# KimmiShi/TorchDistPackage

Measured on AMD Instinct MI355X. Metric: tokens_per_second, higher is better.
Workload: dtype bf16; 1 GPU; model=gpt2_1.3b, global_batch=16, seq_len=1024, parallelism=dp1_pp1_tp1

## Files before the change

torchdistpackage_amd/ops/__init__.py:

```python

from __future__ import annotations

import contextlib
import math
import os
from typing import Optional

import torch

_EXT = None
_EXT_ERR: Optional[str] = None


def _load_extension():
    global _EXT, _EXT_ERR
    if _EXT is not None or _EXT_ERR is not None:
        return _EXT
    import glob
    import importlib.util
    here = os.path.dirname(os.path.abspath(__file__))
    cands = glob.glob(os.path.join(here, "_tdpa_hip*.so"))
    if not cands:
        _EXT_ERR = (f"in-tree HIP extension not found under {here}; "
                    "run `python -m torchdistpackage_amd.ops.build` "
# ... 344 lines not shown
            lse = torch.logsumexp(s, dim=-1)
            p = torch.softmax(s, dim=-1)
            o = torch.matmul(p, vf).to(q.dtype)
        ctx.save_for_backward(q, k, v, o, lse)
        ctx.causal = causal
        ctx.scale = scale
        return o

    @staticmethod
    def backward(ctx, do):
        q, k, v, o, lse = ctx.saved_tensors
        H, Hkv = q.shape[1], k.shape[1]
        rep = H // Hkv
        if q.is_cuda:
            dq = torch.empty(q.shape, dtype=q.dtype, device=q.device)
            dk = torch.empty(q.shape, dtype=k.dtype, device=k.device)
            dv = torch.empty(q.shape, dtype=v.dtype, device=v.device)
            dq, dk, dv = ext("flash_attention").attn_bwd(
                do.contiguous(), q, k, v, o, lse, dq, dk, dv,
                ctx.causal, ctx.scale)
            if rep > 1:
                B, _, S, D = q.shape
                dk = dk.view(B, Hkv, rep, S, D).sum(2).to(k.dtype)
                dv = dv.view(B, Hkv, rep, S, D).sum(2).to(v.dtype)
        else:
            qf = q.float()
            kf = k.float() if rep == 1 else \
                k.float().repeat_interleave(rep, 1)
            vf = v.float() if rep == 1 else \
                v.float().repeat_interleave(rep, 1)
            dof = do.float()
            s = torch.matmul(qf, kf.transpose(-1, -2)) * ctx.scale
            if ctx.causal:
                S = q.shape[-2]
                mask = torch.ones(S, k.shape[-2], dtype=torch.bool,
                                  device=q.device).tril_()
                s = s.masked_fill(~mask, float("-inf"))
            p = torch.softmax(s, dim=-1)
            dv = torch.matmul(p.transpose(-1, -2), dof)
            dp = torch.matmul(dof, vf.transpose(-1, -2))
            d = (dp * p).sum(-1, keepdim=True)
            ds = p * (dp - d) * ctx.scale
            dq = torch.matmul(ds, kf)
            dk = torch.matmul(ds.transpose(-1, -2), qf)
            if rep > 1:
                B, _, S, D = q.shape
                dk = dk.view(B, Hkv, rep, S, D).sum(2)
                dv = dv.view(B, Hkv, rep, S, D).sum(2)
            dq, dk, dv = dq.to(q.dtype), dk.to(k.dtype), dv.to(v.dtype)
        return dq, dk, dv, None, None


_ATTN_KNOBS = ("dq_recompute", "no_tr16", "pstore", "force_v1",
               "max_ds_bytes")


def attention_knobs() -> dict:
    return dict(zip(_ATTN_KNOBS, ext("attention_knobs").attn_knobs()))


@contextlib.contextmanager
def attention_route(**knobs):
    unknown = set(knobs) - set(_ATTN_KNOBS)
    if unknown:
        raise TypeError(f"unknown attention knob(s) {sorted(unknown)}; "
                        f"known: {_ATTN_KNOBS}")
    e = ext("attention_knobs")
    cur = attention_knobs()
    cur.update(knobs)
    prev = e.attn_set_knobs(*(cur[n] for n in _ATTN_KNOBS))
    try:
        yield
    finally:
        e.attn_set_knobs(*prev)


_warned_hd = set()


def flash_attention(q, k, v, causal: bool = True, scale: float = None):
    D = q.shape[-1]
    if q.is_cuda and D not in (64, 128):
        if D not in _warned_hd:
            _warned_hd.add(D)
            print(f"[tdpa.ops] flash_attention: head_dim {D} has no HIP "
                  f"kernel (64/128 do); using composite SDPA for it")
        rep = q.shape[1] // k.shape[1]
        kk = k if rep == 1 else k.repeat_interleave(rep, 1)
        vv = v if rep == 1 else v.repeat_interleave(rep, 1)
        if scale is None:
            scale = 1.0 / math.sqrt(D)
        return torch.nn.functional.scaled_dot_product_attention(
            q, kk, vv, is_causal=causal, scale=scale)
    return _FlashAttentionFn.apply(q, k, v, causal, scale)



def fused_adamw_(param: torch.Tensor, grad: torch.Tensor,
                 exp_avg: torch.Tensor, exp_avg_sq: torch.Tensor,
                 step: int, lr: float, beta1: float, beta2: float,
                 eps: float, weight_decay: float):
    if param.is_cuda:
        ext("fused_adamw").adamw_step(param, grad, exp_avg, exp_avg_sq,
                                      step, lr, beta1, beta2, eps,
                                      weight_decay)
        return
    bc1 = 1 - beta1 ** step
    bc2 = 1 - beta2 ** step
    param.mul_(1 - lr * weight_decay)
    exp_avg.mul_(beta1).add_(grad, alpha=1 - beta1)
    exp_avg_sq.mul_(beta2).addcmul_(grad, grad, value=1 - beta2)
    denom = (exp_avg_sq / bc2).sqrt_().add_(eps)
    param.addcdiv_(exp_avg, denom, value=-lr / bc1)


def ema_update_(ema: torch.Tensor, param: torch.Tensor, decay: float):
    if ema.is_cuda:
        ext("ema_update").ema_update(ema, param.contiguous(), decay)
        return
    ema.lerp_(param.to(ema.dtype), 1.0 - decay)

# ... 381 lines not shown
```

torchdistpackage_amd/ops/csrc/attention.hip:

```cpp

#include <torch/extension.h>
#include <ATen/hip/HIPContext.h>
#include "common.h"
#include "attn_knobs.h"
#include <cstdlib>
#include <string>
#include <tuple>

namespace {

typedef __attribute__((ext_vector_type(8))) __bf16 bf16x8_v;
typedef __attribute__((ext_vector_type(4))) float f32x4;

constexpr int WQ = 16;
constexpr int KT = 32;
constexpr int NW_FWD = 16;
constexpr int NW_DQ = 8;
constexpr int NW_DKDV = 8;

struct Strides {
  long b, h, s;
};

DEVINL bf16x8_v pack8(const unsigned short* p) {
// ... 576 lines not shown
              " must be on q's device ", q.device(), ", got ", t.device());
  TORCH_CHECK(t.scalar_type() == torch::kBFloat16, fn, ": ", name,
              " must be bf16, got ", t.scalar_type());
  TORCH_CHECK(t.dim() == 4 && t.size(0) == B && t.size(1) == Hh &&
                  t.size(2) == S && t.size(3) == D,
              fn, ": ", name, " must be (", B, ", ", Hh, ", ", S, ", ", D,
              "), got ", t.sizes());
  TORCH_CHECK(t.stride(3) == 1, fn, ": ", name,
              " must have a contiguous last dim, got stride ", t.stride(3));
  for (int d = 0; d < 3; ++d)
    TORCH_CHECK(t.size(d) == 1 || t.stride(d) % 8 == 0, fn, ": ", name,
                " stride ", t.stride(d), " of dim ", d, " is not a multiple "
                "of 8 elements: the kernels use 16-byte vector accesses");
  TORCH_CHECK(reinterpret_cast<uintptr_t>(t.data_ptr()) % 16 == 0, fn, ": ",
              name, " is not 16-byte aligned: the kernels use 16-byte vector "
              "accesses");
}

std::tuple<int64_t, int64_t, int64_t, int64_t, int64_t> check_qkv(
    const char* fn, const torch::Tensor& q, const torch::Tensor& k,
    const torch::Tensor& v) {
  TORCH_CHECK(q.is_cuda() && q.scalar_type() == torch::kBFloat16, fn,
              ": bf16 CUDA tensors required");
  TORCH_CHECK(q.dim() == 4, fn, ": q must be (B, H, S, D), got ", q.sizes());
  const int64_t B = q.size(0), H = q.size(1), S = q.size(2), D = q.size(3);
  TORCH_CHECK(D == 64 || D == 128, fn, ": head_dim must be 64 or 128, got ",
              D);
  TORCH_CHECK(B >= 1 && H >= 1 && S >= 1, fn,
              ": empty problem (S = 0?), q is ", q.sizes());
  TORCH_CHECK(k.dim() == 4 && v.dim() == 4, fn,
              ": k and v must be (B, Hkv, S, D), got ", k.sizes(), " and ",
              v.sizes());
  const int64_t Hkv = k.size(1);
  TORCH_CHECK(Hkv >= 1 && H % Hkv == 0, fn,
              ": n_head must be a multiple of n_kv_head, got ", H, " and ",
              Hkv);
  TORCH_CHECK(k.size(2) == S, fn,
              ": cross-attention S_kv != S_q not supported yet (k has ",
              k.size(2), " keys, q ", S, " rows)");
  check_operand(fn, "q", q, q, B, H, S, D);
  check_operand(fn, "k", k, q, B, Hkv, S, D);
  check_operand(fn, "v", v, q, B, Hkv, S, D);
  return {B, H, Hkv, S, D};
}

}

AttnKnobs& attn_knobs_ref() {
  static AttnKnobs k{
      std::getenv("TDPA_DQ_RECOMPUTE") != nullptr,
      std::getenv("TDPA_NO_TR16") != nullptr,
      std::getenv("TDPA_PSTORE") != nullptr,
      std::getenv("TDPA_ATTN_V1") != nullptr,
      (int64_t)4 << 30};
  return k;
}

using KnobTuple = std::tuple<bool, bool, bool, bool, int64_t>;

KnobTuple attn_knobs() {
  const AttnKnobs& k = attn_knobs_ref();
  return {k.dq_recompute, k.no_tr16, k.pstore, k.force_v1, k.max_ds_bytes};
}

KnobTuple attn_set_knobs(bool dq_recompute, bool no_tr16, bool pstore,
                         bool force_v1, int64_t max_ds_bytes) {
  KnobTuple prev = attn_knobs();
  attn_knobs_ref() =
      AttnKnobs{dq_recompute, no_tr16, pstore, force_v1, max_ds_bytes};
  return prev;
}

std::string attn_bwd_route(int64_t B, int64_t H, int64_t S, int64_t D) {
  const AttnBwdRoute r = attn_bwd_select(attn_knobs_ref(), B, H, S, D);
  if (r.v1) return "v1";
  if (r.recompute) return "v2_recompute";
  std::string name = "v2_workspace";
  if (r.pstore) name += "+pstore";
  if (r.no_tr16) name += "+no_tr16";
  return name;
}

void attn_fwd_v2(torch::Tensor q, torch::Tensor k, torch::Tensor v,
                 torch::Tensor o, torch::Tensor lse, bool causal,
                 double scale);
void attn_bwd_dq_v2(torch::Tensor dout, torch::Tensor q, torch::Tensor k,
                    torch::Tensor v, torch::Tensor lse, torch::Tensor delta,
                    torch::Tensor dq, bool causal, double scale);
void attn_bwd_v2_all(torch::Tensor dout, torch::Tensor q, torch::Tensor k,
                     torch::Tensor v, torch::Tensor lse, torch::Tensor delta,
                     torch::Tensor dq, torch::Tensor dk, torch::Tensor dv,
                     bool causal, double scale, const AttnBwdRoute& route);
void attn_bwd_dkdv_v2(torch::Tensor dout, torch::Tensor q, torch::Tensor k,
                      torch::Tensor v, torch::Tensor lse, torch::Tensor delta,
                      torch::Tensor dk, torch::Tensor dv, bool causal,
                      double scale);

std::vector<torch::Tensor> attn_fwd(torch::Tensor q, torch::Tensor k,
                                    torch::Tensor v, torch::Tensor o,
                                    bool causal, double scale) {
  auto [B_, H_, Hkv_, S_, D_] = check_qkv("attn_fwd", q, k, v);
  check_operand("attn_fwd", "o", o, q, B_, H_, S_, D_);
  const int B = B_, H = H_, S = S_, D = D_, Hkv = Hkv_;
  const int q_per_kv = H / Hkv;
  auto lse = torch::empty({B, H, S}, q.options().dtype(torch::kFloat));
  const bool force_v1 = attn_knobs_ref().force_v1;
  if (D == 128 && !force_v1) {
    attn_fwd_v2(q, k, v, o, lse, causal, scale);
    return {o, lse};
  }
  auto stream = at::cuda::getCurrentHIPStream();
  constexpr int QT = NW_FWD * WQ;
  dim3 grid((S + QT - 1) / QT, B * H), block(NW_FWD * 64);
  Strides qs = get_strides(q), ks = get_strides(k), vs = get_strides(v),
          os = get_strides(o);
  const unsigned short* qp = (const unsigned short*)q.data_ptr();
  const unsigned short* kp = (const unsigned short*)k.data_ptr();
  const unsigned short* vp = (const unsigned short*)v.data_ptr();
  unsigned short* op = (unsigned short*)o.data_ptr();
  float* lp = lse.data_ptr<float>();
#define LAUNCH(DD, CC)                                                        \
  hipLaunchKernelGGL((attn_fwd_kernel<DD, CC, NW_FWD>), grid, block, 0,       \
                     stream, qp, kp, vp, op, lp, qs, ks, vs, os, B, H, S,     \
                     (float)scale, q_per_kv)
  if (D == 128) { if (causal) LAUNCH(128, true); else LAUNCH(128, false); }
  else          { if (causal) LAUNCH(64, true);  else LAUNCH(64, false);  }
#undef LAUNCH
  HIP_CHECK_LAST();
  return {o, lse};
}

std::vector<torch::Tensor> attn_bwd(torch::Tensor dout, torch::Tensor q,
                                    torch::Tensor k, torch::Tensor v,
                                    torch::Tensor o, torch::Tensor lse,
                                    torch::Tensor dq, torch::Tensor dk,
                                    torch::Tensor dv,
                                    bool causal, double scale) {
  auto [B_, H_, Hkv_, S_, D_] = check_qkv("attn_bwd", q, k, v);
  const int B = B_, H = H_, S = S_, D = D_, Hkv = Hkv_;
  const int q_per_kv = H / Hkv;
  check_operand("attn_bwd", "dout", dout, q, B, H, S, D);
  check_operand("attn_bwd", "o", o, q, B, H, S, D);
  check_operand("attn_bwd", "dq", dq, q, B, H, S, D);
  TORCH_CHECK(dk.dim() == 4 && dv.dim() == 4 && dk.size(1) == H &&
                  dv.size(1) == H,
// ... 2 lines not shown
  check_operand("attn_bwd", "dk", dk, q, B, H, S, D);
  check_operand("attn_bwd", "dv", dv, q, B, H, S, D);
  TORCH_CHECK(lse.is_cuda() && lse.device() == q.device() &&
                  lse.scalar_type() == torch::kFloat && lse.dim() == 3 &&
                  lse.size(0) == B && lse.size(1) == H && lse.size(2) == S &&
                  lse.is_contiguous(),
              "attn_bwd: lse must be a contiguous fp32 (", B, ", ", H, ", ",
              S, ") tensor on q's device, got ", lse.scalar_type(), " ",
              lse.sizes(), " strides ", lse.strides(), " on ", lse.device());
  auto delta = torch::empty({B, H, S}, q.options().dtype(torch::kFloat));
  auto stream = at::cuda::getCurrentHIPStream();
  Strides qs = get_strides(q), ks = get_strides(k), vs = get_strides(v),
          os = get_strides(o), dos = get_strides(dout),
          dqs = get_strides(dq), dks = get_strides(dk), dvs = get_strides(dv);

  launch_attn_delta(o, dout, delta, os, dos, B, H, S, D, stream);

  const AttnBwdRoute route = attn_bwd_select(attn_knobs_ref(), B, H, S, D);
  if (!route.v1) {
    attn_bwd_v2_all(dout, q, k, v, lse, delta, dq, dk, dv, causal, scale,
                    route);
    HIP_CHECK_LAST();
    return {dq, dk, dv};
  }
  constexpr int QT_DQ = NW_DQ * WQ;
  constexpr int QT_KV = NW_DKDV * WQ;
  dim3 grid_dq((S + QT_DQ - 1) / QT_DQ, B * H), block_dq(NW_DQ * 64);
  dim3 grid_kv((S + QT_KV - 1) / QT_KV, B * H), block_kv(NW_DKDV * 64);
  const unsigned short* qp = (const unsigned short*)q.data_ptr();
  const unsigned short* kp = (const unsigned short*)k.data_ptr();
  const unsigned short* vp = (const unsigned short*)v.data_ptr();
  const unsigned short* dop = (const unsigned short*)dout.data_ptr();
  const float* lp = lse.data_ptr<float>();
  const float* delp = delta.data_ptr<float>();
#define LAUNCH_BWD(DD, CC)                                                    \
  do {                                                                        \
    hipLaunchKernelGGL((attn_bwd_dq_kernel<DD, CC, NW_DQ>), grid_dq,         \
                       block_dq, 0, stream, qp, kp, vp, dop, lp, delp,        \
                       (unsigned short*)dq.data_ptr(), qs, ks, vs, dos, dqs,  \
                       B, H, S, (float)scale, q_per_kv);                      \
    hipLaunchKernelGGL((attn_bwd_dkdv_kernel<DD, CC, NW_DKDV>), grid_kv,      \
                       block_kv, 0, stream, qp, kp, vp, dop, lp, delp,        \
                       (unsigned short*)dk.data_ptr(),                        \
                       (unsigned short*)dv.data_ptr(), qs, ks, vs, dos,       \
                       dks, dvs, B, H, S, (float)scale, q_per_kv);            \
  } while (0)
  if (D == 128) { if (causal) LAUNCH_BWD(128, true); else LAUNCH_BWD(128, false); }
  else          { if (causal) LAUNCH_BWD(64, true);  else LAUNCH_BWD(64, false);  }
#undef LAUNCH_BWD
  HIP_CHECK_LAST();
  return {dq, dk, dv};
}

torch::Tensor attn_delta(torch::Tensor o, torch::Tensor dout) {
  TORCH_CHECK(o.is_cuda() && o.scalar_type() == torch::kBFloat16 &&
                  o.dim() == 4,
              "attn_delta: o must be a (B, H, S, D) bf16 device tensor");
  const int64_t B = o.size(0), H = o.size(1), S = o.size(2), D = o.size(3);
  TORCH_CHECK(D == 64 || D == 128,
              "attn_delta: head_dim must be 64 or 128, got ", D);
  TORCH_CHECK(B >= 1 && H >= 1 && S >= 1, "attn_delta: empty problem, o is ",
              o.sizes());
  check_operand("attn_delta", "o", o, o, B, H, S, D);
  check_operand("attn_delta", "dout", dout, o, B, H, S, D);
  auto delta = torch::empty({B, H, S}, o.options().dtype(torch::kFloat));
  launch_attn_delta(o, dout, delta, get_strides(o), get_strides(dout), (int)B,
                    (int)H, (int)S, (int)D, at::cuda::getCurrentHIPStream());
  HIP_CHECK_LAST();
  return delta;
}
```

torchdistpackage_amd/ops/csrc/attention_v2.hip:

```cpp

#include <torch/extension.h>
#include <ATen/hip/HIPContext.h>
#include "common.h"
#include "attn_knobs.h"

namespace {

typedef __attribute__((ext_vector_type(8))) __bf16 bf16x8_v;
typedef __attribute__((ext_vector_type(16))) float f32x16;

constexpr int D2 = 128;
constexpr int QW = 32;
constexpr int NW2 = 8;
constexpr int QT2 = NW2 * QW;
constexpr int KV = 64;

struct Strides2 {
  long b, h, s;
};

DEVINL bf16x8_v pack8v(const unsigned short* p) {
  return *(const bf16x8_v*)p;
}

// ... 700 lines not shown
      }
    }
  }
}

}

void attn_bwd_dkdv_v2(torch::Tensor dout, torch::Tensor q, torch::Tensor k,
                      torch::Tensor v, torch::Tensor lse, torch::Tensor delta,
                      torch::Tensor dk, torch::Tensor dv, bool causal,
                      double scale) {
  const int B = q.size(0), H = q.size(1), S = q.size(2), D = q.size(3);
  const int Hkv = k.size(1);
  const int q_per_kv = H / Hkv;
  TORCH_CHECK(D == 128);
  auto get = [](const torch::Tensor& t) {
    return Strides2{t.stride(0), t.stride(1), t.stride(2)};
  };
  auto stream = at::cuda::getCurrentHIPStream();
  dim3 grid((S + QT2 - 1) / QT2, B * H), block(512);
#define L_KV2(CC, WDS, DSP, SPAD, PW, PM1, PM2)                               \
  do {                                                                        \
    hipLaunchKernelGGL((attn_bwd_dkdv_v2_kernel<CC, false, false, PM1>),      \
                       grid, block, 0,                                        \
                       stream, (const unsigned short*)q.data_ptr(),           \
                       (const unsigned short*)k.data_ptr(),                   \
                       (const unsigned short*)v.data_ptr(),                   \
                       (const unsigned short*)dout.data_ptr(),                \
                       lse.data_ptr<float>(), delta.data_ptr<float>(),        \
                       (unsigned short*)dv.data_ptr(), nullptr, 0, PW,        \
                       get(q),                                                \
                       get(k), get(v), get(dout), get(dv), B, H, S,           \
                       (float)scale, q_per_kv);                               \
    hipLaunchKernelGGL((attn_bwd_dkdv_v2_kernel<CC, true, WDS, PM2>),         \
                       grid, block, 0,                                        \
                       stream, (const unsigned short*)q.data_ptr(),           \
                       (const unsigned short*)k.data_ptr(),                   \
                       (const unsigned short*)v.data_ptr(),                   \
                       (const unsigned short*)dout.data_ptr(),                \
                       lse.data_ptr<float>(), delta.data_ptr<float>(),        \
                       (unsigned short*)dk.data_ptr(), DSP, SPAD, PW,         \
                       get(q),                                                \
                       get(k), get(v), get(dout), get(dk), B, H, S,           \
                       (float)scale, q_per_kv);                               \
  } while (0)
  if (causal) L_KV2(true, false, nullptr, 0, nullptr, 0, 0);
  else L_KV2(false, false, nullptr, 0, nullptr, 0, 0);
  HIP_CHECK_LAST();
}


namespace {

template <bool CAUSAL>
__launch_bounds__(512)
__global__ void attn_bwd_dq_lite_kernel(
    const unsigned short* __restrict__ k,
    const unsigned short* __restrict__ dsb,
    unsigned short* __restrict__ dq,
    Strides2 ks, Strides2 dqs,
    int B, int H, int S, long spad, int q_per_kv) {
  __shared__ __attribute__((aligned(16))) unsigned short kt_lds[2][D2 * KV];

  const int bh = blockIdx.y;
  const int bb = bh / H, hh = bh % H;
  const int hkv = hh / q_per_kv;
  const int qtile = CAUSAL ? (gridDim.x - 1 - blockIdx.x) : blockIdx.x;
  const int qbase = qtile * QT2;
  if (qbase >= S) return;
  const int tid = threadIdx.x;
  const int wid = tid / WAVE;
  const int lane = tid % WAVE;
  const int l31 = lane & 31;
  const int hi = lane >> 5;

  const unsigned short* kp = k + bb * ks.b + hkv * ks.h;
  const int qrow = qbase + wid * QW + l31;
  const unsigned short* dsp = dsb +
      ((long)bh * S + (qrow < S ? qrow : S - 1)) * spad;

  f32x16 acc[4];
#pragma unroll
  for (int ds = 0; ds < 4; ++ds) acc[ds] = (f32x16)(0.f);

  const int kv_end = CAUSAL ? min(S, qbase + QT2) : S;

  bf16x8_v k_reg[2];
  auto load_regs = [&](int kt0) {
#pragma unroll
    for (int c = 0; c < 2; ++c) {
      int idx = tid * 8 + c * 4096;
      int gkey = kt0 + idx / D2;
      k_reg[c] = gkey < S ? pack8v(kp + (long)gkey * ks.s + idx % D2)
                          : (bf16x8_v)(__bf16)0.f;
    }
  };
  auto stage_kt = [&](int b) {
#pragma unroll
    for (int c = 0; c < 2; ++c) {
      int idx = tid * 8 + c * 4096;
      int key = idx / D2;
      int col = idx % D2;
      const unsigned short* ksrc = (const unsigned short*)&k_reg[c];
#pragma unroll
      for (int j = 0; j < 8; ++j)
        kt_lds[b][swzV(col + j, key)] = ksrc[j];
// ... 136 lines not shown
#pragma unroll
    for (int ds = 0; ds < 4; ++ds) {
#pragma unroll
      for (int kt = 0; kt < 2; ++kt) {
#pragma unroll
        for (int kc = 0; kc < 2; ++kc) {
          unsigned long long lo, hic;
          const unsigned off = (unsigned)(ds * 4096 +
                                          (kt * 32 + kc * 16) * 32);
          asm volatile(
              "ds_read_b64_tr_b16 %0, %2 offset:%3\n\t"
              "ds_read_b64_tr_b16 %1, %2 offset:%4\n\t"
              "s_waitcnt lgkmcnt(0)"
              : "=v"(lo), "=v"(hic)
              : "v"(abase + off), "i"(0), "i"(128));
          bf16x8_v a_kt;
          ((unsigned long long*)&a_kt)[0] = lo;
          ((unsigned long long*)&a_kt)[1] = hic;
          acc[ds] = __builtin_amdgcn_mfma_f32_32x32x16_bf16(
              a_kt, db[kt][kc], acc[ds], 0, 0, 0);
        }
      }
    }

    if (kt0 + KV < kv_end) {
      stage_img(buf ^ 1);
      if (kt0 + 2 * KV < kv_end) load_regs(kt0 + 2 * KV);
    }
    __syncthreads();
    buf ^= 1;
  }

  if (qrow < S) {
    unsigned short* dqp = dq + bb * dqs.b + hh * dqs.h + (long)qrow * dqs.s;
#pragma unroll
    for (int ds = 0; ds < 4; ++ds) {
#pragma unroll
      for (int blk = 0; blk < 4; ++blk) {
        int d0 = ds * 32 + 8 * blk + 4 * hi;
        unsigned short out4[4];
#pragma unroll
        for (int j = 0; j < 4; ++j)
          out4[j] = f2bf(acc[ds][4 * blk + j]);
        *(ushort4*)(dqp + d0) = *(ushort4*)out4;
      }
    }
  }
}

}

AttnBwdRoute attn_bwd_select(const AttnKnobs& knobs, int64_t B, int64_t H,
                             int64_t S, int64_t D) {
  AttnBwdRoute r{false, false, false, false};
  r.v1 = D != 128 || knobs.force_v1;
  if (r.v1) return r;
  const int64_t spad_est = (S + QT2 - 1) / QT2 * QT2;
  const int64_t pmul = knobs.pstore ? 4 : 2;
  const int64_t ds_bytes = B * H * S * spad_est * pmul;
  r.recompute = knobs.dq_recompute || ds_bytes > knobs.max_ds_bytes;
  if (r.recompute) return r;
  r.pstore = knobs.pstore;
  r.no_tr16 = knobs.no_tr16;
  return r;
}

void attn_bwd_v2_all(torch::Tensor dout, torch::Tensor q, torch::Tensor k,
                     torch::Tensor v, torch::Tensor lse, torch::Tensor delta,
                     torch::Tensor dq, torch::Tensor dk, torch::Tensor dv,
                     bool causal, double scale, const AttnBwdRoute& route) {
  TORCH_CHECK(!route.v1, "attn_bwd_v2_all: the v1 route is attn_bwd's");
  if (route.recompute) {
    attn_bwd_dq_v2(dout, q, k, v, lse, delta, dq, causal, scale);
    attn_bwd_dkdv_v2(dout, q, k, v, lse, delta, dk, dv, causal, scale);
    return;
  }
  const int B = q.size(0), H = q.size(1), S = q.size(2), D = q.size(3);
  const int Hkv = k.size(1);
  const int q_per_kv = H / Hkv;
  TORCH_CHECK(D == 128);
  auto get = [](const torch::Tensor& t) {
    return Strides2{t.stride(0), t.stride(1), t.stride(2)};
  };
  auto stream = at::cuda::getCurrentHIPStream();
  dim3 grid((S + QT2 - 1) / QT2, B * H), block(512);
  const long spad = (long)grid.x * QT2;
  auto dsw = torch::empty({(long)B * H, (long)S, spad}, q.options());
  unsigned short* dsp = (unsigned short*)dsw.data_ptr();
  const bool pstore = route.pstore;
  torch::Tensor pwt;
  unsigned short* pw = nullptr;
  if (pstore) {
    pwt = torch::empty({(long)B * H, spad, spad}, q.options());
    pw = (unsigned short*)pwt.data_ptr();
  }
  if (causal) {
    if (pw) L_KV2(true, true, dsp, spad, pw, 1, 2);
    else L_KV2(true, true, dsp, spad, nullptr, 0, 0);
  } else {
    if (pw) L_KV2(false, true, dsp, spad, pw, 1, 2);
    else L_KV2(false, true, dsp, spad, nullptr, 0, 0);
  }
#undef L_KV2
  const bool no_tr16 = route.no_tr16;
#define L_DQL(CC)                                                             \
  do {                                                                        \
    if (no_tr16)                                                              \
      hipLaunchKernelGGL((attn_bwd_dq_lite_kernel<CC>), grid, block, 0,       \
                         stream, (const unsigned short*)k.data_ptr(), dsp,    \
                         (unsigned short*)dq.data_ptr(), get(k), get(dq),     \
                         B, H, S, spad, q_per_kv);                            \
    else                                                                      \
      hipLaunchKernelGGL((attn_bwd_dq_lite_tr_kernel<CC>), grid, block, 0,    \
                         stream, (const unsigned short*)k.data_ptr(), dsp,    \
                         (unsigned short*)dq.data_ptr(), get(k), get(dq),     \
                         B, H, S, spad, q_per_kv);                            \
  } while (0)
  if (causal) L_DQL(true); else L_DQL(false);
#undef L_DQL
  HIP_CHECK_LAST();
}
```

torchdistpackage_amd/ops/csrc/attn_knobs.h:

```cpp
#pragma once

#include <cstdint>

struct AttnKnobs {
  bool dq_recompute;
  bool no_tr16;
  bool pstore;
  bool force_v1;
  int64_t max_ds_bytes;
};

AttnKnobs& attn_knobs_ref();

struct AttnBwdRoute {
  bool v1, recompute, pstore, no_tr16;
};

AttnBwdRoute attn_bwd_select(const AttnKnobs& knobs, int64_t B, int64_t H,
                             int64_t S, int64_t D);

constexpr float kAttnPFlush = 0x1p-40f;
```

torchdistpackage_amd/ops/csrc/bindings.cpp:

```cpp
#include <torch/extension.h>

#include "grouped_gemm_plan.h"

std::vector<torch::Tensor> rmsnorm_fwd(torch::Tensor x, torch::Tensor w,
                                       double eps);
std::vector<torch::Tensor> rmsnorm_bwd(torch::Tensor dy, torch::Tensor x,
                                       torch::Tensor w, torch::Tensor rstd);
std::vector<torch::Tensor> layernorm_fwd(torch::Tensor x, torch::Tensor w,
                                         torch::Tensor b, double eps);
std::vector<torch::Tensor> layernorm_bwd(torch::Tensor dy, torch::Tensor x,
                                         torch::Tensor w, torch::Tensor mean,
                                         torch::Tensor rstd);
torch::Tensor bias_gelu_fwd(torch::Tensor x, torch::Tensor bias);
torch::Tensor bias_gelu_bwd(torch::Tensor dy, torch::Tensor x,
                            torch::Tensor bias);
void adamw_step(torch::Tensor p, torch::Tensor g, torch::Tensor m,
                torch::Tensor v, long step, double lr, double beta1,
                double beta2, double eps, double wd);
void multi_adamw_step(torch::Tensor cpid, torch::Tensor coff,
                      torch::Tensor pptrs, torch::Tensor gptrs,
                      torch::Tensor mptrs, torch::Tensor moffs,
                      torch::Tensor numels,
                      torch::Tensor m, torch::Tensor v,
                      long step, double lr, double beta1, double beta2,
                      double eps, double wd, bool param_bf16, bool grad_bf16);
void adamw_step_dev(torch::Tensor p, torch::Tensor g, torch::Tensor m,
                    torch::Tensor v, torch::Tensor coef, double beta1,
                    double beta2, double eps);
void adamw_prelude(torch::Tensor step, torch::Tensor hyp, torch::Tensor coef);
void multi_adamw_step_dev(torch::Tensor cpid, torch::Tensor coff,
                          torch::Tensor pptrs, torch::Tensor gptrs,
                          torch::Tensor mptrs, torch::Tensor moffs,
                          torch::Tensor numels,
                          torch::Tensor m, torch::Tensor v,
                          torch::Tensor coef, double beta1, double beta2,
                          double eps, bool param_bf16, bool grad_bf16);
void ema_update(torch::Tensor ema, torch::Tensor p, double decay);
torch::Tensor l2norm_sq(torch::Tensor x);
void scale_inplace(torch::Tensor x, double s);
std::vector<torch::Tensor> attn_fwd(torch::Tensor q, torch::Tensor k,
                                    torch::Tensor v, torch::Tensor o,
                                    bool causal, double scale);
std::vector<torch::Tensor> attn_bwd(torch::Tensor dout, torch::Tensor q,
                                    torch::Tensor k, torch::Tensor v,
                                    torch::Tensor o, torch::Tensor lse,
                                    torch::Tensor dq, torch::Tensor dk,
                                    torch::Tensor dv,
                                    bool causal, double scale);
std::tuple<bool, bool, bool, bool, int64_t> attn_knobs();
std::tuple<bool, bool, bool, bool, int64_t> attn_set_knobs(
    bool dq_recompute, bool no_tr16, bool pstore, bool force_v1,
    int64_t max_ds_bytes);
std::string attn_bwd_route(int64_t B, int64_t H, int64_t S, int64_t D);
torch::Tensor mfma_probe_16x16x32(torch::Tensor a, torch::Tensor b);
torch::Tensor mfma_probe_32x32x16(torch::Tensor a, torch::Tensor b);
torch::Tensor tr16_probe(long addr_mode);
std::vector<torch::Tensor> ce_fwd(torch::Tensor logits, torch::Tensor targets);
torch::Tensor gemm_fprop(torch::Tensor x, torch::Tensor w,
                         c10::optional<torch::Tensor> bias);
torch::Tensor rope_apply(torch::Tensor x, torch::Tensor cs, torch::Tensor sn,
                         long pos0, bool fwd);
torch::Tensor swiglu_fwd(torch::Tensor a, torch::Tensor b);
torch::Tensor bgelu_b_fwd(torch::Tensor x, torch::Tensor bias);
torch::Tensor bgelu_b_bwd(torch::Tensor dy, torch::Tensor x,
                          torch::Tensor bias);
std::vector<torch::Tensor> swiglu_bwd(torch::Tensor dy, torch::Tensor a,
                                      torch::Tensor b);
torch::Tensor gemm_dgrad(torch::Tensor dy, torch::Tensor w, bool kswz);
torch::Tensor gemm_wgrad(torch::Tensor dy, torch::Tensor x, long splitk,
                         bool kswz);
torch::Tensor ce_bwd(torch::Tensor logits, torch::Tensor targets,
                     torch::Tensor lse, torch::Tensor grad_out);
std::vector<torch::Tensor> ce_partial_fwd(torch::Tensor logits,
                                          torch::Tensor targets);
torch::Tensor gemv_bf16(torch::Tensor x, torch::Tensor W,
                        c10::optional<torch::Tensor> bias);
torch::Tensor gemv_w8a16(torch::Tensor x, torch::Tensor q,
                         torch::Tensor scale,
                         c10::optional<torch::Tensor> bias);
torch::Tensor rope_apply_pos(torch::Tensor x, torch::Tensor cs,
                             torch::Tensor sn, torch::Tensor pos, bool fwd);
torch::Tensor decode_attention(torch::Tensor q, torch::Tensor k_cache,
                               torch::Tensor v_cache, torch::Tensor out,
                               c10::optional<torch::Tensor> pos_t, long pos0,
                               double scale, long split_kv);
torch::Tensor grouped_gemm_fprop(torch::Tensor x, torch::Tensor w,
                                 torch::Tensor offs,
                                 c10::optional<torch::Tensor> bias);
torch::Tensor grouped_gemm_dgrad(torch::Tensor dy, torch::Tensor w,
                                 torch::Tensor offs);
std::tuple<torch::Tensor, c10::optional<torch::Tensor>> grouped_gemm_wgrad(
    torch::Tensor dy, torch::Tensor x, torch::Tensor offs,
    bool want_bias_grad);
torch::Tensor grouped_gemm_plan(torch::Tensor offs_cpu, int64_t T);
std::vector<torch::Tensor> bias_residual_layernorm_fwd(
    torch::Tensor y, c10::optional<torch::Tensor> bias, torch::Tensor x_res,
    torch::Tensor ln_w, torch::Tensor ln_b, double eps);
std::vector<torch::Tensor> layernorm_bwd_residual(
    torch::Tensor dh, torch::Tensor x, torch::Tensor w, torch::Tensor mean,
    torch::Tensor rstd, torch::Tensor g_res, bool want_colsum);
std::vector<torch::Tensor> bias_gelu_bwd_colsum(torch::Tensor dy,
                                                torch::Tensor x,
                                                torch::Tensor bias);
bool bias_gelu_bwd_colsum_ok(int64_t D);
int64_t fused_ln_max_d();
torch::Tensor bias_residual_add(torch::Tensor y,
                                c10::optional<torch::Tensor> bias,
                                torch::Tensor x_res);
torch::Tensor attn_delta(torch::Tensor o, torch::Tensor dout);

PYBIND11_MODULE(TORCH_EXTENSION_NAME, m) {
  m.def("rmsnorm_fwd", &rmsnorm_fwd);
  m.def("rmsnorm_bwd", &rmsnorm_bwd);
  m.def("layernorm_fwd", &layernorm_fwd);
  m.def("layernorm_bwd", &layernorm_bwd);
  m.def("bias_gelu_fwd", &bias_gelu_fwd);
  m.def("bias_gelu_bwd", &bias_gelu_bwd);
  m.def("adamw_step", &adamw_step);
  m.def("multi_adamw_step", &multi_adamw_step);
  m.def("adamw_step_dev", &adamw_step_dev);
  m.def("adamw_prelude", &adamw_prelude);
  m.def("multi_adamw_step_dev", &multi_adamw_step_dev);
  m.def("ema_update", &ema_update);
  m.def("l2norm_sq", &l2norm_sq);
  m.def("scale_inplace", &scale_inplace);
  m.def("attn_fwd", &attn_fwd);
  m.def("attn_bwd", &attn_bwd);
  m.def("attn_knobs", &attn_knobs,
        "(dq_recompute, no_tr16, pstore, force_v1, max_ds_bytes)");
  m.def("attn_set_knobs", &attn_set_knobs,
        "set the five attention knobs; returns the previous five");
  m.def("attn_bwd_route", &attn_bwd_route,
        "name of the backward route for (B, H, S, D) under the current knobs");
  m.def("mfma_probe_16x16x32", &mfma_probe_16x16x32);
  m.def("mfma_probe_32x32x16", &mfma_probe_32x32x16);
  m.def("tr16_probe", &tr16_probe);
  m.def("ce_fwd", &ce_fwd);
  m.def("gemm_fprop", &gemm_fprop);
  m.def("rope_apply", &rope_apply);
  m.def("swiglu_fwd", &swiglu_fwd);
  m.def("bgelu_b_fwd", &bgelu_b_fwd);
  m.def("bgelu_b_bwd", &bgelu_b_bwd);
  m.def("swiglu_bwd", &swiglu_bwd);
  m.def("gemm_dgrad", &gemm_dgrad);
  m.def("gemm_wgrad", &gemm_wgrad);
  m.def("ce_bwd", &ce_bwd);
  m.def("ce_partial_fwd", &ce_partial_fwd);
  m.def("gemv_bf16", &gemv_bf16);
  m.def("gemv_w8a16", &gemv_w8a16);
  m.def("rope_apply_pos", &rope_apply_pos);
  m.def("decode_attention", &decode_attention);
  m.def("grouped_gemm_fprop", &grouped_gemm_fprop);
  m.def("grouped_gemm_dgrad", &grouped_gemm_dgrad);
  m.def("grouped_gemm_wgrad", &grouped_gemm_wgrad);
  m.def("grouped_gemm_plan", &grouped_gemm_plan,
        "(offs_cpu, T) -> (row-tile bound, 3) int64: (expert, first row, "
        "row count) per block, expert -1 = idle");
  m.attr("GROUPED_GEMM_BM") = GG_BM;
  m.def("bias_residual_layernorm_fwd", &bias_residual_layernorm_fwd,
        "(y, bias|None, x_res, ln_w, ln_b, eps) -> (x_new, h, mean, rstd)");
  m.def("layernorm_bwd_residual", &layernorm_bwd_residual,
        "(dh, x, w, mean, rstd, g_res, want_colsum) -> (g, partial): "
        "fp32 (2|3, grid, D); partial[k].sum(0), one sum per slice, = dw, db"
        "[, colsum(g)] (one sum(1) would change the bits of dw and db)");
  m.def("bias_gelu_bwd_colsum", &bias_gelu_bwd_colsum,
        "(dy, x, bias) -> (dx, partial): partial.sum(0) = colsum(dx) in fp32");
  m.def("fused_ln_max_d", &fused_ln_max_d,
        "widest last dim of the fused LayerNorm kernels");
  m.def("bias_gelu_bwd_colsum_ok", &bias_gelu_bwd_colsum_ok,
        "whether bias_gelu_bwd_colsum covers last dim D");
  m.def("bias_residual_add", &bias_residual_add,
        "(y, bias|None, x_res) -> bf16(x_res + bf16(y + bias))");
  m.def("attn_delta", &attn_delta,
        "(o, dout) (B, H, S, D) bf16 -> rowsum(o * dout) (B, H, S) fp32");
}
```

torchdistpackage_amd/parallel/tensor/tp_utils.py:

```python

from __future__ import annotations

from typing import Optional

import torch
import torch.distributed as dist
import torch.nn as nn
import torch.nn.functional as F

from ...ops.gemm import linear as fast_linear

_TP_GROUP: Optional[dist.ProcessGroup] = None


def set_tp_group(group: Optional[dist.ProcessGroup]):
    global _TP_GROUP
    _TP_GROUP = group


def get_tp_group() -> Optional[dist.ProcessGroup]:
    global _TP_GROUP
    if _TP_GROUP is None:
        try:
            from ...dist.topo import tpc
# ... 25 lines not shown
def _all_gather_first_dim(x: torch.Tensor) -> torch.Tensor:
    tp = get_tp_size()
    if tp == 1:
        return x
    group = get_tp_group()
    out_shape = list(x.shape)
    out_shape[0] *= tp
    out = torch.empty(out_shape, dtype=x.dtype, device=x.device)
    dist.all_gather_into_tensor(out, x.contiguous(), group=group)
    return out


def _reduce_scatter_first_dim(x: torch.Tensor) -> torch.Tensor:
    tp = get_tp_size()
    if tp == 1:
        return x
    group = get_tp_group()
    assert x.shape[0] % tp == 0, \
        f"first dim {x.shape[0]} not divisible by tp {tp}"
    out_shape = list(x.shape)
    out_shape[0] //= tp
    x = x.contiguous()
    if _backend_is_gloo(group):
        x = x.clone()
        dist.all_reduce(x, group=group)
        r = dist.get_rank(group)
        return x.narrow(0, r * out_shape[0], out_shape[0]).clone()
    out = torch.empty(out_shape, dtype=x.dtype, device=x.device)
    dist.reduce_scatter_tensor(out, x, group=group)
    return out


def _split_first_dim(x: torch.Tensor) -> torch.Tensor:
    tp = get_tp_size()
    if tp == 1:
        return x
    r = get_tp_rank()
    n = x.shape[0] // tp
    return x.narrow(0, r * n, n).contiguous()


def _all_reduce(x: torch.Tensor) -> torch.Tensor:
    if get_tp_size() == 1:
        return x
    dist.all_reduce(x, group=get_tp_group())
    return x



class _ReduceFromTp(torch.autograd.Function):

    @staticmethod
    def forward(ctx, x):
        return _all_reduce(x.clone())

    @staticmethod
    def backward(ctx, grad):
        return grad


class _CopyToTp(torch.autograd.Function):

    @staticmethod
    def forward(ctx, x):
        return x

    @staticmethod
    def backward(ctx, grad):
        return _all_reduce(grad.contiguous().clone())


class _ReduceScatterToSp(torch.autograd.Function):

    @staticmethod
    def forward(ctx, x):
        return _reduce_scatter_first_dim(x)

    @staticmethod
    def backward(ctx, grad):
        return _all_gather_first_dim(grad.contiguous())


class _GatherFromSp(torch.autograd.Function):

    @staticmethod
    def forward(ctx, x, bwd_mode: str = "reduce_scatter"):
        ctx.bwd_mode = bwd_mode
        return _all_gather_first_dim(x)

    @staticmethod
    def backward(ctx, grad):
        grad = grad.contiguous()
        if ctx.bwd_mode == "split":
            return _split_first_dim(grad), None
        return _reduce_scatter_first_dim(grad), None


def reduce_from_tp_region(x):
    return _ReduceFromTp.apply(x)


def copy_to_tp_region(x):
    return _CopyToTp.apply(x)


def reduce_scatter_to_sequence_parallel_region(x):
    out = _ReduceScatterToSp.apply(x)
    set_sequence_parallel_attr(out)
    return out


def gather_from_sequence_parallel_region(x, bwd_mode: str = "reduce_scatter"):
    return _GatherFromSp.apply(x, bwd_mode)



def set_sequence_parallel_attr(t: torch.Tensor):
    t.sequence_parallel = True


def is_sequence_parallel(t: torch.Tensor) -> bool:
# ... 169 lines not shown
```

Measured before the change: 109,200 tokens/s.

## Fuse dK/dV backward into single-pass kernel and skip TP clones at size one

Adds a fused attention backward kernel for head dim 128 that computes S and dP, then accumulates both dK and dV in one pass over query tiles. It uses double-buffered LDS staging and transposed LDS reads, and optionally writes dS for the dQ pass. This becomes the default dK/dV route unless pstore, no_tr16 or a new split_dkdv knob selects the old two-pass kernels. Separately, the tensor-parallel reduce and copy functions no longer clone activations and gradients when the TP group has size one, which removes a copy per call. The new kernel carries a large register footprint from eight accumulators plus the V fragments, which may limit occupancy.

```diff
diff --git a/torchdistpackage_amd/ops/__init__.py b/torchdistpackage_amd/ops/__init__.py
--- a/torchdistpackage_amd/ops/__init__.py
+++ b/torchdistpackage_amd/ops/__init__.py
@@ -420,11 +420,14 @@
 
 
 _ATTN_KNOBS = ("dq_recompute", "no_tr16", "pstore", "force_v1",
-               "max_ds_bytes")
-
-
-def attention_knobs() -> dict:
-    return dict(zip(_ATTN_KNOBS, ext("attention_knobs").attn_knobs()))
+               "max_ds_bytes", "split_dkdv")
+
+
+def attention_knobs(extended: bool = False) -> dict:
+    cur = dict(zip(_ATTN_KNOBS, ext("attention_knobs").attn_knobs()))
+    if not extended:
+        cur = {n: cur[n] for n in _ATTN_KNOBS[:5]}
+    return cur
 
 
 @contextlib.contextmanager
@@ -434,7 +437,7 @@
         raise TypeError(f"unknown attention knob(s) {sorted(unknown)}; "
                         f"known: {_ATTN_KNOBS}")
     e = ext("attention_knobs")
-    cur = attention_knobs()
+    cur = attention_knobs(extended=True)
     cur.update(knobs)
     prev = e.attn_set_knobs(*(cur[n] for n in _ATTN_KNOBS))
     try:
diff --git a/torchdistpackage_amd/ops/csrc/attention.hip b/torchdistpackage_amd/ops/csrc/attention.hip
--- a/torchdistpackage_amd/ops/csrc/attention.hip
+++ b/torchdistpackage_amd/ops/csrc/attention.hip
@@ -652,32 +652,35 @@
       std::getenv("TDPA_NO_TR16") != nullptr,
       std::getenv("TDPA_PSTORE") != nullptr,
       std::getenv("TDPA_ATTN_V1") != nullptr,
-      (int64_t)4 << 30};
+      (int64_t)4 << 30,
+      std::getenv("TDPA_SPLIT_DKDV") != nullptr};
   return k;
 }
 
-using KnobTuple = std::tuple<bool, bool, bool, bool, int64_t>;
+using KnobTuple = std::tuple<bool, bool, bool, bool, int64_t, bool>;
 
 KnobTuple attn_knobs() {
   const AttnKnobs& k = attn_knobs_ref();
-  return {k.dq_recompute, k.no_tr16, k.pstore, k.force_v1, k.max_ds_bytes};
+  return {k.dq_recompute, k.no_tr16, k.pstore, k.force_v1, k.max_ds_bytes,
+          k.split_dkdv};
 }
 
 KnobTuple attn_set_knobs(bool dq_recompute, bool no_tr16, bool pstore,
-                         bool force_v1, int64_t max_ds_bytes) {
+                         bool force_v1, int64_t max_ds_bytes,
+                         bool split_dkdv) {
   KnobTuple prev = attn_knobs();
-  attn_knobs_ref() =
-      AttnKnobs{dq_recompute, no_tr16, pstore, force_v1, max_ds_bytes};
+  attn_knobs_ref() = AttnKnobs{dq_recompute, no_tr16,      pstore,
+                               force_v1,     max_ds_bytes, split_dkdv};
   return prev;
 }
 
 std::string attn_bwd_route(int64_t B, int64_t H, int64_t S, int64_t D) {
   const AttnBwdRoute r = attn_bwd_select(attn_knobs_ref(), B, H, S, D);
   if (r.v1) return "v1";
-  if (r.recompute) return "v2_recompute";
-  std::string name = "v2_workspace";
+  std::string name = r.recompute ? "v2_recompute" : "v2_workspace";
   if (r.pstore) name += "+pstore";
   if (r.no_tr16) name += "+no_tr16";
+  if (r.split_dkdv) name += "+split_dkdv";
   return name;
 }
 
@@ -690,7 +693,8 @@
 void attn_bwd_v2_all(torch::Tensor dout, torch::Tensor q, torch::Tensor k,
                      torch::Tensor v, torch::Tensor lse, torch::Tensor delta,
                      torch::Tensor dq, torch::Tensor dk, torch::Tensor dv,
-                     bool causal, double scale, const AttnBwdRoute& route);
+                     bool causal, double scale, const AttnBwdRoute& route,
+                     bool skip_dq = false);
 void attn_bwd_dkdv_v2(torch::Tensor dout, torch::Tensor q, torch::Tensor k,
                       torch::Tensor v, torch::Tensor lse, torch::Tensor delta,
                       torch::Tensor dk, torch::Tensor dv, bool causal,
@@ -799,6 +803,28 @@
   return {dq, dk, dv};
 }
 
+void attn_bwd_dkdv(torch::Tensor dout, torch::Tensor q, torch::Tensor k,
+                   torch::Tensor v, torch::Tensor lse, torch::Tensor delta,
+                   torch::Tensor dk, torch::Tensor dv, bool causal,
+                   double scale) {
+  auto [B, H, Hkv, S, D] = check_qkv("attn_bwd_dkdv", q, k, v);
+  (void)Hkv;
+  check_operand("attn_bwd_dkdv", "dout", dout, q, B, H, S, D);
+  check_operand("attn_bwd_dkdv", "dk", dk, q, B, H, S, D);
+  check_operand("attn_bwd_dkdv", "dv", dv, q, B, H, S, D);
+  for (const torch::Tensor* t : {&lse, &delta})
+    TORCH_CHECK(t->is_cuda() && t->device() == q.device() &&
+                    t->scalar_type() == torch::kFloat && t->dim() == 3 &&
+                    t->size(0) == B && t->size(1) == H && t->size(2) == S &&
+                    t->is_contiguous(),
+                "attn_bwd_dkdv: lse and delta must be contiguous fp32 (", B,
+                ", ", H, ", ", S, ") tensors on q's device");
+  const AttnBwdRoute route = attn_bwd_select(attn_knobs_ref(), B, H, S, D);
+  TORCH_CHECK(!route.v1, "attn_bwd_dkdv: head dim 128 on the v2 route only");
+  attn_bwd_v2_all(dout, q, k, v, lse, delta, torch::Tensor(), dk, dv, causal,
+                  scale, route, true);
+}
+
 torch::Tensor attn_delta(torch::Tensor o, torch::Tensor dout) {
   TORCH_CHECK(o.is_cuda() && o.scalar_type() == torch::kBFloat16 &&
                   o.dim() == 4,
diff --git a/torchdistpackage_amd/ops/csrc/attention_v2.hip b/torchdistpackage_amd/ops/csrc/attention_v2.hip
--- a/torchdistpackage_amd/ops/csrc/attention_v2.hip
+++ b/torchdistpackage_amd/ops/csrc/attention_v2.hip
@@ -776,6 +776,285 @@
 
 namespace {
 
+typedef __attribute__((ext_vector_type(4))) __bf16 bf16x4_v;
+typedef __attribute__((address_space(3))) bf16x4_v lds_bf16x4;
+typedef __attribute__((address_space(3))) bf16x8_v lds_bf16x8;
+
+DEVINL int swzT(int row, int ch) {
+  return row * (D2 * 2) + ((ch ^ (((row & 3) << 2) | ((row >> 2) & 3))) << 4);
+}
+
+template <bool CAUSAL, bool WRITE_DS>
+__launch_bounds__(512)
+__global__ void attn_bwd_dkdv_fused_v2_kernel(
+    const unsigned short* __restrict__ q,
+    const unsigned short* __restrict__ k,
+    const unsigned short* __restrict__ v,
+    const unsigned short* __restrict__ dout,
+    const float* __restrict__ lse,
+    const float* __restrict__ delta,
+    unsigned short* __restrict__ dk,
+    unsigned short* __restrict__ dv,
+    unsigned short* __restrict__ ds_out, long spad,
+    Strides2 qs, Strides2 ks, Strides2 vs, Strides2 dos, Strides2 dks,
+    Strides2 dvs, int B, int H, int S, float scale, int q_per_kv) {
+  struct Images {
+    unsigned short q[2][KV * D2];
+    unsigned short dO[2][KV * D2];
+    unsigned short k[QT2 * D2];
+  };
+  __shared__ __attribute__((aligned(256))) Images img;
+  constexpr unsigned kTile = KV * D2 * 2;
+  constexpr unsigned kDoOff = 2 * kTile;
+  __shared__ float lse_lds[2][KV];
+  __shared__ float del_lds[2][KV];
+
+  const int bh = blockIdx.y;
+  const int bb = bh / H, hh = bh % H;
+  const int hkv = hh / q_per_kv;
+  const int kbase = blockIdx.x * QT2;
+  if (kbase >= S) return;
+  const int tid = threadIdx.x;
+  const int wid = tid / WAVE;
+  const int lane = tid % WAVE;
+  const int l31 = lane & 31;
+  const int hi = lane >> 5;
+
+  const unsigned short* qp = q + bb * qs.b + hh * qs.h;
+  const unsigned short* kp = k + bb * ks.b + hkv * ks.h;
+  const unsigned short* vp = v + bb * vs.b + hkv * vs.h;
+  const unsigned short* dop = dout + bb * dos.b + hh * dos.h;
+  const float* lsep = lse + (long)bh * S;
+  const float* delp = delta + (long)bh * S;
+
+  const int key = kbase + wid * QW + l31;
+  bf16x8_v vt_frag[8];
+  {
+    long r = (long)(key < S ? key : S - 1);
+#pragma unroll
+    for (int c = 0; c < 8; ++c)
+      vt_frag[c] = pack8v(vp + r * vs.s + c * 16 + hi * 8);
+  }
+#pragma unroll
+  for (int c = 0; c < 8; ++c) {
+    int idx = tid * 8 + c * 4096;
+    int row = idx / D2;
+    int col = idx % D2;
+    int grow = kbase + row;
+    long r = (long)(grow < S ? grow : S - 1);
+    *(bf16x8_v*)((char*)img.k + swzT(row, col >> 3)) =
+        pack8v(kp + r * ks.s + col);
+  }
+  const unsigned img_base = (unsigned)(unsigned long long)
+      (__attribute__((address_space(3))) unsigned short*)&img.q[0][0];
+  const unsigned row_lane = img_base + (unsigned)swzT(l31, hi);
+  const unsigned krow_lane = row_lane + 2 * kDoOff + wid * (QW * D2 * 2);
+
+  const int tq = (lane >> 2) & 3;
+  const int tp = lane & 3;
+  const int tg1 = (lane >> 4) & 1;
+  const unsigned tr_lane = img_base +
+      (unsigned)((hi * 8 + tq) * (D2 * 2) +
+                 (((tq << 2) | ((tg1 ^ hi) << 1) | (tp >> 1)) << 4) +
+                 (tp & 1) * 8);
+  auto tr_addr = [&](unsigned tl, int qt, int kc, int sub,
+                     int ds) -> unsigned {
+    return (tl ^ (unsigned)((((ds << 2) | sub)) << 4)) +
+           (unsigned)((qt * 32 + kc * 16 + sub * 4) * (D2 * 2));
+  };
+
+  f32x16 acc_dk[4], acc_dv[4];
+#pragma unroll
+  for (int ds = 0; ds < 4; ++ds) {
+    acc_dk[ds] = (f32x16)(0.f);
+    acc_dv[ds] = (f32x16)(0.f);
+  }
+
+  const int qt_start = CAUSAL ? kbase : 0;
+
+  auto stage = [&](int qt0, int b) {
+    int st = tid;
+    asm volatile("" : "+v"(st));
+#pragma unroll
+    for (int c = 0; c < 2; ++c) {
+      int idx = st * 8 + c * 4096;
+      int row = idx / D2;
+      int col = idx % D2;
+      int grow = qt0 + row;
+      long gr = (long)(grow < S ? grow : S - 1);
+      bf16x8_v qv = pack8v(qp + gr * qs.s + col);
+      bf16x8_v dv8 = pack8v(dop + gr * dos.s + col);
+      if (grow >= S) {
+        qv = (bf16x8_v)(__bf16)0.f;
+        dv8 = (bf16x8_v)(__bf16)0.f;
+      }
+      const int off = swzT(row, col >> 3);
+      *(bf16x8_v*)((char*)&img.q[b][0] + off) = qv;
+      *(bf16x8_v*)((char*)&img.dO[b][0] + off) = dv8;
+    }
+    if (tid < KV) {
+      int grow = qt0 + tid;
+      int gr = grow < S ? grow : S - 1;
+      float l = lsep[gr], d = delp[gr];
+      lse_lds[b][tid] = grow < S ? l : 0.f;
+      del_lds[b][tid] = grow < S ? d : 0.f;
+    }
+  };
+  stage(qt_start, 0);
+  __syncthreads();
+
+  auto make_frag = [&](const f32x16& x, int kc, bf16x8_v& fb) {
+    int m0 = 2 * kc, m1 = 2 * kc + 1;
+    unsigned a0 = cvt_pk_bf16(x[4 * m0], x[4 * m0 + 1]);
+    unsigned a1 = cvt_pk_bf16(x[4 * m0 + 2], x[4 * m0 + 3]);
+    unsigned b0 = cvt_pk_bf16(x[4 * m1], x[4 * m1 + 1]);
+    unsigned b1 = cvt_pk_bf16(x[4 * m1 + 2], x[4 * m1 + 3]);
+    auto s0 = __builtin_amdgcn_permlane32_swap(a0, b0, false, false);
+    auto s1 = __builtin_amdgcn_permlane32_swap(a1, b1, false, false);
+    unsigned* dst = (unsigned*)&fb;
+    if (hi == 0) {
+      dst[0] = a0; dst[1] = a1; dst[2] = s0[1]; dst[3] = s1[1];
+    } else {
+      dst[0] = s0[0]; dst[1] = s1[0]; dst[2] = b0; dst[3] = b1;
+    }
+  };
+  auto tr_frag = [&](unsigned tl, unsigned img_off, int qt, int kc, int ds) {
+    bf16x4_v lo = __builtin_amdgcn_ds_read_tr16_b64_v4bf16(
+        (lds_bf16x4*)(tr_addr(tl, qt, kc, 0, ds) + img_off));
+    bf16x4_v hi4 = __builtin_amdgcn_ds_read_tr16_b64_v4bf16(
+        (lds_bf16x4*)(tr_addr(tl, qt, kc, 1, ds) + img_off));
+    return __builtin_shufflevector(lo, hi4, 0, 1, 2, 3, 4, 5, 6, 7);
+  };
+  auto row_frag = [&](unsigned addr) {
+    return *(const lds_bf16x8*)addr;
+  };
+
+  int buf = 0;
+  for (int qt0 = qt_start; qt0 < S; qt0 += KV) {
+    unsigned rl = row_lane + (unsigned)buf * kTile;
+    unsigned tl = tr_lane + (unsigned)buf * kTile;
+    unsigned kl = krow_lane;
+    asm volatile("" : "+v"(rl), "+v"(tl), "+v"(kl));
+
+#pragma unroll
+    for (int qt = 0; qt < 2; ++qt) {
+      __builtin_amdgcn_sched_barrier(0);
+      f32x16 s_acc = (f32x16)(0.f);
+      f32x16 dp_acc = (f32x16)(0.f);
+#pragma unroll
+      for (int c = 0; c < 8; ++c) {
+        const unsigned ra = (rl ^ (unsigned)(c << 5)) +
+                            (unsigned)(qt * 32 * D2 * 2);
+        bf16x8_v a_q = row_frag(ra);
+        bf16x8_v b_k = row_frag(kl ^ (unsigned)(c << 5));
+        s_acc = __builtin_amdgcn_mfma_f32_32x32x16_bf16(
+            a_q, b_k, s_acc, 0, 0, 0);
+        bf16x8_v a_do = row_frag(ra + kDoOff);
+        dp_acc = __builtin_amdgcn_mfma_f32_32x32x16_bf16(
+            a_do, vt_frag[c], dp_acc, 0, 0, 0);
+      }
+
+      __builtin_amdgcn_sched_group_barrier(0x100, 6, 0);
+#pragma unroll
+      for (int c = 0; c < 6; ++c) {
+        __builtin_amdgcn_sched_group_barrier(0x008, 2, 0);
+        __builtin_amdgcn_sched_group_barrier(0x100, 3, 0);
+      }
+      __builtin_amdgcn_sched_group_barrier(0x008, 4, 0);
+      __builtin_amdgcn_sched_barrier(0);
+
+      bf16x8_v fp[2], fds[2];
+#pragma unroll
+      for (int kc = 0; kc < 2; ++kc) {
+#pragma unroll
+        for (int r = 8 * kc; r < 8 * kc + 8; ++r) {
+          int qrel = qt * 32 + (r & 3) + 8 * (r >> 2) + 4 * hi;
+          int qrow = qt0 + qrel;
+          const bool valid = key < S && qrow < S && (!CAUSAL || key <= qrow);
+          const float e = __expf(s_acc[r] * scale - lse_lds[buf][qrel]);
+          const float p = valid ? e : 0.f;
+          const float pf = (valid && !(e < kAttnPFlush)) ? e : 0.f;
+          s_acc[r] = p * (dp_acc[r] - del_lds[buf][qrel]) * scale;
+          dp_acc[r] = pf;
+          if (WRITE_DS && qrow < S)
+            ds_out[((long)bh * S + qrow) * spad + key] = f2bf(s_acc[r]);
+        }
+        make_frag(dp_acc, kc, fp[kc]);
+        make_frag(s_acc, kc, fds[kc]);
+        __builtin_amdgcn_sched_barrier(0);
+      }
+
+#pragma unroll
+      for (int ds = 0; ds < 4; ++ds) {
+#pragma unroll
+        for (int kc = 0; kc < 2; ++kc) {
+          acc_dv[ds] = __builtin_amdgcn_mfma_f32_32x32x16_bf16(
+              tr_frag(tl, kDoOff, qt, kc, ds), fp[kc], acc_dv[ds], 0, 0, 0);
+          acc_dk[ds] = __builtin_amdgcn_mfma_f32_32x32x16_bf16(
+              tr_frag(tl, 0, qt, kc, ds), fds[kc], acc_dk[ds], 0, 0, 0);
+        }
+      }
+    }
+
+    if (qt0 + KV < S) stage(qt0 + KV, buf ^ 1);
+    __syncthreads();
+    buf ^= 1;
+  }
+
+  if (key < S) {
+    unsigned short* okp = dk + bb * dks.b + hh * dks.h + (long)key * dks.s;
+    unsigned short* ovp = dv + bb * dvs.b + hh * dvs.h + (long)key * dvs.s;
+#pragma unroll
+    for (int ds = 0; ds < 4; ++ds) {
+#pragma unroll
+      for (int blk = 0; blk < 4; ++blk) {
+        int d0 = ds * 32 + 8 * blk + 4 * hi;
+        unsigned short k4[4], v4[4];
+#pragma unroll
+        for (int j = 0; j < 4; ++j) {
+          k4[j] = f2bf(acc_dk[ds][4 * blk + j]);
+          v4[j] = f2bf(acc_dv[ds][4 * blk + j]);
+        }
+        *(ushort4*)(okp + d0) = *(ushort4*)k4;
+        *(ushort4*)(ovp + d0) = *(ushort4*)v4;
+      }
+    }
+  }
+}
+
+void launch_dkdv_fused(torch::Tensor& dout, torch::Tensor& q, torch::Tensor& k,
+                       torch::Tensor& v, torch::Tensor& lse,
+                       torch::Tensor& delta, torch::Tensor& dk,
+                       torch::Tensor& dv, unsigned short* ds_ws, long spad,
+                       bool causal, double scale) {
+  const int B = q.size(0), H = q.size(1), S = q.size(2);
+  const int q_per_kv = H / (int)k.size(1);
+  auto get = [](const torch::Tensor& t) {
+    return Strides2{t.stride(0), t.stride(1), t.stride(2)};
+  };
+  auto stream = at::cuda::getCurrentHIPStream();
+  dim3 grid((S + QT2 - 1) / QT2, B * H), block(512);
+#define L_FUSED(CC, WDS)                                                      \
+  hipLaunchKernelGGL((attn_bwd_dkdv_fused_v2_kernel<CC, WDS>), grid, block,   \
+                     0, stream, (const unsigned short*)q.data_ptr(),          \
+                     (const unsigned short*)k.data_ptr(),                     \
+                     (const unsigned short*)v.data_ptr(),                     \
+                     (const unsigned short*)dout.data_ptr(),                  \
+                     lse.data_ptr<float>(), delta.data_ptr<float>(),          \
+                     (unsigned short*)dk.data_ptr(),                          \
+                     (unsigned short*)dv.data_ptr(), ds_ws, spad, get(q),     \
+                     get(k), get(v), get(dout), get(dk), get(dv), B, H, S,    \
+                     (float)scale, q_per_kv)
+  if (ds_ws) { if (causal) L_FUSED(true, true); else L_FUSED(false, true); }
+  else { if (causal) L_FUSED(true, false); else L_FUSED(false, false); }
+#undef L_FUSED
+}
+
+}
+
+
+namespace {
+
 template <bool CAUSAL>
 __launch_bounds__(512)
 __global__ void attn_bwd_dq_lite_kernel(
@@ -1018,27 +1297,37 @@
 
 AttnBwdRoute attn_bwd_select(const AttnKnobs& knobs, int64_t B, int64_t H,
                              int64_t S, int64_t D) {
-  AttnBwdRoute r{false, false, false, false};
+  AttnBwdRoute r{false, false, false, false, false};
   r.v1 = D != 128 || knobs.force_v1;
   if (r.v1) return r;
   const int64_t spad_est = (S + QT2 - 1) / QT2 * QT2;
   const int64_t pmul = knobs.pstore ? 4 : 2;
   const int64_t ds_bytes = B * H * S * spad_est * pmul;
   r.recompute = knobs.dq_recompute || ds_bytes > knobs.max_ds_bytes;
+  r.split_dkdv = knobs.split_dkdv;
   if (r.recompute) return r;
   r.pstore = knobs.pstore;
   r.no_tr16 = knobs.no_tr16;
+  if (r.pstore || r.no_tr16) r.split_dkdv = false;
   return r;
 }
 
 void attn_bwd_v2_all(torch::Tensor dout, torch::Tensor q, torch::Tensor k,
                      torch::Tensor v, torch::Tensor lse, torch::Tensor delta,
                      torch::Tensor dq, torch::Tensor dk, torch::Tensor dv,
-                     bool causal, double scale, const AttnBwdRoute& route) {
+                     bool causal, double scale, const AttnBwdRoute& route,
+                     bool skip_dq) {
   TORCH_CHECK(!route.v1, "attn_bwd_v2_all: the v1 route is attn_bwd's");
   if (route.recompute) {
-    attn_bwd_dq_v2(dout, q, k, v, lse, delta, dq, causal, scale);
-    attn_bwd_dkdv_v2(dout, q, k, v, lse, delta, dk, dv, causal, scale);
+    if (!skip_dq) attn_bwd_dq_v2(dout, q, k, v, lse, delta, dq, causal, scale);
+    if (route.two_pass()) {
+      attn_bwd_dkdv_v2(dout, q, k, v, lse, delta, dk, dv, causal, scale);
+    } else {
+      TORCH_CHECK(q.size(3) == 128);
+      launch_dkdv_fused(dout, q, k, v, lse, delta, dk, dv, nullptr, 0, causal,
+                        scale);
+      HIP_CHECK_LAST();
+    }
     return;
   }
   const int B = q.size(0), H = q.size(1), S = q.size(2), D = q.size(3);
@@ -1060,7 +1349,10 @@
     pwt = torch::empty({(long)B * H, spad, spad}, q.options());
     pw = (unsigned short*)pwt.data_ptr();
   }
-  if (causal) {
+  if (!route.two_pass()) {
+    launch_dkdv_fused(dout, q, k, v, lse, delta, dk, dv, dsp, spad, causal,
+                      scale);
+  } else if (causal) {
     if (pw) L_KV2(true, true, dsp, spad, pw, 1, 2);
     else L_KV2(true, true, dsp, spad, nullptr, 0, 0);
   } else {
@@ -1068,6 +1360,10 @@
     else L_KV2(false, true, dsp, spad, nullptr, 0, 0);
   }
 #undef L_KV2
+  if (skip_dq) {
+    HIP_CHECK_LAST();
+    return;
+  }
   const bool no_tr16 = route.no_tr16;
 #define L_DQL(CC)                                                             \
   do {                                                                        \
diff --git a/torchdistpackage_amd/ops/csrc/attn_knobs.h b/torchdistpackage_amd/ops/csrc/attn_knobs.h
--- a/torchdistpackage_amd/ops/csrc/attn_knobs.h
+++ b/torchdistpackage_amd/ops/csrc/attn_knobs.h
@@ -8,12 +8,14 @@
   bool pstore;
   bool force_v1;
   int64_t max_ds_bytes;
+  bool split_dkdv;
 };
 
 AttnKnobs& attn_knobs_ref();
 
 struct AttnBwdRoute {
-  bool v1, recompute, pstore, no_tr16;
+  bool v1, recompute, pstore, no_tr16, split_dkdv;
+  bool two_pass() const { return pstore || no_tr16 || split_dkdv; }
 };
 
 AttnBwdRoute attn_bwd_select(const AttnKnobs& knobs, int64_t B, int64_t H,
diff --git a/torchdistpackage_amd/ops/csrc/bindings.cpp b/torchdistpackage_amd/ops/csrc/bindings.cpp
--- a/torchdistpackage_amd/ops/csrc/bindings.cpp
+++ b/torchdistpackage_amd/ops/csrc/bindings.cpp
@@ -47,10 +47,10 @@
                                     torch::Tensor dq, torch::Tensor dk,
                                     torch::Tensor dv,
                                     bool causal, double scale);
-std::tuple<bool, bool, bool, bool, int64_t> attn_knobs();
-std::tuple<bool, bool, bool, bool, int64_t> attn_set_knobs(
+std::tuple<bool, bool, bool, bool, int64_t, bool> attn_knobs();
+std::tuple<bool, bool, bool, bool, int64_t, bool> attn_set_knobs(
     bool dq_recompute, bool no_tr16, bool pstore, bool force_v1,
-    int64_t max_ds_bytes);
+    int64_t max_ds_bytes, bool split_dkdv);
 std::string attn_bwd_route(int64_t B, int64_t H, int64_t S, int64_t D);
 torch::Tensor mfma_probe_16x16x32(torch::Tensor a, torch::Tensor b);
 torch::Tensor mfma_probe_32x32x16(torch::Tensor a, torch::Tensor b);
@@ -108,6 +108,10 @@
                                 c10::optional<torch::Tensor> bias,
                                 torch::Tensor x_res);
 torch::Tensor attn_delta(torch::Tensor o, torch::Tensor dout);
+void attn_bwd_dkdv(torch::Tensor dout, torch::Tensor q, torch::Tensor k,
+                   torch::Tensor v, torch::Tensor lse, torch::Tensor delta,
+                   torch::Tensor dk, torch::Tensor dv, bool causal,
+                   double scale);
 
 PYBIND11_MODULE(TORCH_EXTENSION_NAME, m) {
   m.def("rmsnorm_fwd", &rmsnorm_fwd);
@@ -127,9 +131,9 @@
   m.def("attn_fwd", &attn_fwd);
   m.def("attn_bwd", &attn_bwd);
   m.def("attn_knobs", &attn_knobs,
-        "(dq_recompute, no_tr16, pstore, force_v1, max_ds_bytes)");
+        "(dq_recompute, no_tr16, pstore, force_v1, max_ds_bytes, split_dkdv)");
   m.def("attn_set_knobs", &attn_set_knobs,
-        "set the five attention knobs; returns the previous five");
+        "set the six attention knobs; returns the previous six");
   m.def("attn_bwd_route", &attn_bwd_route,
         "name of the backward route for (B, H, S, D) under the current knobs");
   m.def("mfma_probe_16x16x32", &mfma_probe_16x16x32);
@@ -173,4 +177,7 @@
         "(y, bias|None, x_res) -> bf16(x_res + bf16(y + bias))");
   m.def("attn_delta", &attn_delta,
         "(o, dout) (B, H, S, D) bf16 -> rowsum(o * dout) (B, H, S) fp32");
+  m.def("attn_bwd_dkdv", &attn_bwd_dkdv,
+        "(dout, q, k, v, lse, delta, dk, dv, causal, scale): the dk/dv stage "
+        "of the head-dim-128 backward alone, under the current knobs");
 }
diff --git a/torchdistpackage_amd/parallel/tensor/tp_utils.py b/torchdistpackage_amd/parallel/tensor/tp_utils.py
--- a/torchdistpackage_amd/parallel/tensor/tp_utils.py
+++ b/torchdistpackage_amd/parallel/tensor/tp_utils.py
@@ -101,6 +101,8 @@
 
     @staticmethod
     def forward(ctx, x):
+        if get_tp_size() == 1:
+            return x
         return _all_reduce(x.clone())
 
     @staticmethod
@@ -116,6 +118,8 @@
 
     @staticmethod
     def backward(ctx, grad):
+        if get_tp_size() == 1:
+            return grad
         return _all_reduce(grad.contiguous().clone())
 
 
```

After: 113,000 tokens/s (median of 6 runs). 1.03x the previous value.
